# HKU-BAL/Clair3-RNA

Hardware: AMD Instinct MI355X
Metric: candidate sites/sec (tensor build + inference) (higher is better)
Workload: dtype f16 hi/lo split x3, f32 accumulate (fp32-equivalent); 1 GPU; synthetic ONT dRNA004 chr20 ~20x (BASELINE.json configs[1]); contig_len=64444167, chunks=13, channels=18, precision=f16x3, reads_per_rank=53937, exonic_bp_per_rank=1936903, parallelism=chunks sharded by contig, 1 rank(s), no collective, streams=2

## Files before the change

### clair3_rna_amd/csrc/net_kernels.hpp

```cpp
#pragma once
#include <hip/hip_runtime.h>
#include <mutex>
#include <chrono>
#include <type_traits>
#include <stdint.h>

#include <cmath>
#include <cstring>
#include <functional>
#include <string>
#include <vector>

#include "../../include/c3r.h"

namespace c3r {

typedef float floatx16 __attribute__((ext_vector_type(16)));
typedef float floatx4 __attribute__((ext_vector_type(4)));

constexpr int NET_H1 = 128;
constexpr int NET_H2 = 160;
constexpr int NET_T = C3R_WINDOW;
constexpr int NET_SITES = 32;
constexpr int LSTM_SB = 2;
constexpr int LSTM_SITES = NET_SITES * LSTM_SB;
#ifndef C3R_W8_PD
#define C3R_W8_PD 1
#endif
#ifndef C3R_W8_MAP
#define C3R_W8_MAP 0
#endif
#ifndef C3R_W8_PRIO
#define C3R_W8_PRIO 0
#endif
#ifndef C3R_DIR_ILV
#define C3R_DIR_ILV 1
#endif
#ifndef C3R_Y1_NT_LOAD
#define C3R_Y1_NT_LOAD 1
#endif
#ifndef C3R_Y1_NT_STORE
#define C3R_Y1_NT_STORE 1
#endif
#ifndef C3R_L2_SKIP0
#define C3R_L2_SKIP0 1
#endif
#define C3R_Y1_AUX (C3R_Y1_NT_LOAD ? 2 : 0)
template <class V, class P>
__device__ __forceinline__ void y1_store(V v, P p) {
    if constexpr (C3R_Y1_NT_STORE) __builtin_nontemporal_store(v, p);
    else *p = v;
}
constexpr int NET_FLAT = NET_T * 2 * NET_H2;
constexpr int NET_L4 = 128;

__device__ __forceinline__ float fast_sigmoid(float x) {
    return __builtin_amdgcn_rcpf(1.0f + __builtin_amdgcn_exp2f(-1.4426950408889634f * x));
}
__device__ __forceinline__ float fast_tanh(float x) {
    return fmaf(2.0f, __builtin_amdgcn_rcpf(1.0f + __builtin_amdgcn_exp2f(-2.8853900817779268f * x)), -1.0f);
}
__device__ __forceinline__ float gate_frac(float a, float b) {
    const float t = 1.0f + a;
    const float r = __builtin_amdgcn_rcpf(fmaf(t, b, t));
    return fmaf(-b, r, r);
}
__device__ __forceinline__ float cell_fence(float x) {
    asm("" : "+v"(x));
    return x;
}
typedef _Float16 half2v __attribute__((ext_vector_type(2)));
typedef float float2v __attribute__((ext_vector_type(2)));
__device__ __forceinline__ void split_h2(float h0, float h1, half2v &hi, half2v &lo, float &d0, float &d1) {
    asm("" : "+v"(h0));
    asm("" : "+v"(h1));
    const float2v h = {h0, h1};
    hi = __builtin_convertvector(h, half2v);
    asm("v_fma_mix_f32 %0, -%1, 1.0, %2 op_sel_hi:[1,1,0]" : "=v"(d0) : "v"(hi), "v"(h0));
    asm("v_fma_mix_f32 %0, -%1, 1.0, %2 op_sel:[1,0,0] op_sel_hi:[1,1,0]" : "=v"(d1) : "v"(hi), "v"(h1));
    const float2v d = {d0, d1};
    lo = __builtin_convertvector(d, half2v);
}
__device__ __forceinline__ float selu(float x) {
    const float scale = 1.0507009873554805f, alpha = 1.6732632423543772f;
    return x > 0.f ? scale * x : scale * alpha * (__expf(x) - 1.0f);
}

template <int INP, int CIN, int H, bool INT_IN, int SB = 2, int ABL = 0>
__global__ __launch_bounds__(256, (SB == 1 ? 2 : 1)) void k_lstm(const void *__restrict__ xin, const float4 *__restrict__ Wp,
                                                                  const float *__restrict__ bp, float *__restrict__ y, int n,
                                                                  const int32_t *__restrict__ row_idx = nullptr ,
                                                                  int x16 = 0 ) {
    constexpr int NGX = INP / 8;
    constexpr int NGH = H / 8;
    constexpr int NG = NGX + NGH;
    constexpr int HP = H + 4;
    constexpr int NBLK = 4 * H / 32;
    constexpr int NT = NBLK / 4;
    constexpr int WG_SITES = 32 * SB;
    static_assert(INP % 16 == 0 && H % 32 == 0, "shape: even k-group counts for the ping-pong pipeline");
    __shared__ __attribute__((aligned(16))) float hbuf[2][WG_SITES][HP];

    const int tid = threadIdx.x, lane = tid & 63, wave = tid >> 6;
    const int j = lane & 31, hh = lane >> 5;
    const int dir = blockIdx.y;
    const int site0 = blockIdx.x * WG_SITES;

    const float4 *wl = Wp + ((size_t)(dir * 4 + wave) * NG) * NT * 64 + lane;
    float bias_a[NT];
#pragma unroll
    for (int tt = 0; tt < NT; ++tt) bias_a[tt] = hh == 0 ? bp[((size_t)dir * NBLK + wave * NT + tt) * 32 + j] : 0.f;

    float cst[NT][SB][4];
#pragma unroll
    for (int tt = 0; tt < NT; ++tt)
#pragma unroll
        for (int sb = 0; sb < SB; ++sb)
#pragma unroll
            for (int q = 0; q < 4; ++q) cst[tt][sb][q] = 0.f;

    for (int i = tid; i < WG_SITES * HP; i += 256) (&hbuf[0][0][0])[i] = 0.f;
    __syncthreads();

    size_t xoff[SB];
#pragma unroll
    for (int sb = 0; sb < SB; ++sb) {
        int sj = site0 + 32 * sb + j;
        if (sj >= n) sj = n - 1;
        if (INT_IN && row_idx) sj = row_idx[sj];
        xoff[sb] = (size_t)sj * NET_T * CIN;
    }

    for (int step = 0; step < NET_T; ++step) {
        const int t = dir ? NET_T - 1 - step : step;
        const int cur = step & 1, nxt = cur ^ 1;

        auto ldx = [&](int g, float4 (&b)[SB]) {
#pragma unroll
            for (int sb = 0; sb < SB; ++sb) {
                if (ABL & 16) { b[sb] = make_float4(1.f, 0.5f, 0.25f, (float)g); continue; }
                if (INT_IN) {
                    const int k0 = 8 * g + 4 * hh;
                    if (x16) {
                        const int16_t *xp = (const int16_t *)xin + xoff[sb] + (size_t)t * CIN;
                        b[sb].x = (k0 + 0 < CIN) ? (float)xp[k0 + 0] : 0.f;
                        b[sb].y = (k0 + 1 < CIN) ? (float)xp[k0 + 1] : 0.f;
                        b[sb].z = (k0 + 2 < CIN) ? (float)xp[k0 + 2] : 0.f;
                        b[sb].w = (k0 + 3 < CIN) ? (float)xp[k0 + 3] : 0.f;
                    } else {
                        const int32_t *xp = (const int32_t *)xin + xoff[sb] + (size_t)t * CIN;
                        b[sb].x = (k0 + 0 < CIN) ? (float)xp[k0 + 0] : 0.f;
                        b[sb].y = (k0 + 1 < CIN) ? (float)xp[k0 + 1] : 0.f;
                        b[sb].z = (k0 + 2 < CIN) ? (float)xp[k0 + 2] : 0.f;
                        b[sb].w = (k0 + 3 < CIN) ? (float)xp[k0 + 3] : 0.f;
                    }
                } else {
                    b[sb] = *(const float4 *)((const float *)xin + xoff[sb] + (size_t)t * CIN + 8 * g + 4 * hh);
                }
            }
        };
        auto ldh = [&](int g, float4 (&b)[SB]) {
#pragma unroll
            for (int sb = 0; sb < SB; ++sb) b[sb] = *(const float4 *)&hbuf[cur][32 * sb + j][8 * g + 4 * hh];
        };
        auto ldw = [&](int g, float4 (&a)[NT]) {
            const float4 *wg = wl + (size_t)((ABL & 1) ? 0 : g) * NT * 64;
#pragma unroll
            for (int tt = 0; tt < NT; ++tt) a[tt] = wg[tt * 64];
        };

        floatx16 acc[NT][SB];
        {
            floatx16 z;
#pragma unroll
            for (int r = 0; r < 16; ++r) z[r] = 0.f;
#pragma unroll
            for (int tt = 0; tt < NT; ++tt)
#pragma unroll
                for (int sb = 0; sb < SB; ++sb) acc[tt][sb] = __builtin_amdgcn_mfma_f32_32x32x2f32(bias_a[tt], 1.0f, z, 0, 0, 0);
        }
#define C3R_MMA_K(comp)                                                                                              \
    _Pragma("unroll") for (int tt = 0; tt < NT; ++tt) _Pragma("unroll") for (int sb = 0; sb < SB; ++sb)             \
        acc[tt][sb] = __builtin_amdgcn_mfma_f32_32x32x2f32(a[tt].comp, b[sb].comp, acc[tt][sb], 0, 0, 0);
        auto mma = [&](const float4 (&a)[NT], const float4 (&b)[SB]) {
            C3R_MMA_K(x) C3R_MMA_K(y) C3R_MMA_K(z) C3R_MMA_K(w)
        };
#undef C3R_MMA_K
        float4 a0[NT], a1[NT], b0[SB], b1[SB];
#define C3R_FENCE() __builtin_amdgcn_sched_barrier(0)
        ldw(0, a0);
        ldx(0, b0);
#pragma unroll 1
        for (int g = 0; g + 2 < NGX; g += 2) {
            C3R_FENCE(); ldw(g + 1, a1); ldx(g + 1, b1); C3R_FENCE();
            mma(a0, b0);
            C3R_FENCE(); ldw(g + 2, a0); ldx(g + 2, b0); C3R_FENCE();
            mma(a1, b1);
        }
        C3R_FENCE(); ldw(NGX - 1, a1); ldx(NGX - 1, b1); C3R_FENCE();
        mma(a0, b0);
        C3R_FENCE(); ldw(NGX, a0); ldh(0, b0); C3R_FENCE();
        mma(a1, b1);
#pragma unroll 1
        for (int g = 0; g + 2 < NGH; g += 2) {
            C3R_FENCE(); ldw(NGX + g + 1, a1); ldh(g + 1, b1); C3R_FENCE();
            mma(a0, b0);
            C3R_FENCE(); ldw(NGX + g + 2, a0); ldh(g + 2, b0); C3R_FENCE();
            mma(a1, b1);
        }
        C3R_FENCE(); ldw(NG - 1, a1); ldh(NGH - 1, b1); C3R_FENCE();
        mma(a0, b0);
        mma(a1, b1);
        C3R_FENCE();
#undef C3R_FENCE
#pragma unroll
        for (int tt = 0; tt < NT; ++tt) {
#pragma unroll
            for (int sb = 0; sb < SB; ++sb) {
                float hq[4];
#pragma unroll
                for (int q = 0; q < 4; ++q) {
                    if (ABL & 2) { hq[q] = acc[tt][sb][4 * q] + acc[tt][sb][4 * q + 1] + acc[tt][sb][4 * q + 2] + acc[tt][sb][4 * q + 3]; continue; }
                    const float ig = fast_sigmoid(acc[tt][sb][4 * q + 0]);
                    const float fg = fast_sigmoid(acc[tt][sb][4 * q + 1]);
                    const float gg = fast_tanh(acc[tt][sb][4 * q + 2]);
                    const float og = fast_sigmoid(acc[tt][sb][4 * q + 3]);
                    const float c = fg * cst[tt][sb][q] + ig * gg;
                    cst[tt][sb][q] = c;
                    hq[q] = og * fast_tanh(c);
                }
                *(float4 *)&hbuf[nxt][32 * sb + j][8 * (wave * NT + tt) + 4 * hh] = make_float4(hq[0], hq[1], hq[2], hq[3]);
            }
        }
        if (!(ABL & 8)) __syncthreads();
        constexpr int HV = H / 4;
        if (!(ABL & 4))
        for (int f = tid; f < WG_SITES * HV; f += 256) {
            const int row = f / HV, c4 = f % HV;
            const int s = site0 + row;
            if (s < n) {
                const float4 v = *(const float4 *)&hbuf[nxt][row][4 * c4];
                *(float4 *)(y + ((size_t)s * NET_T + t) * (2 * H) + dir * H + 4 * c4) = v;
            }
        }
    }
}

typedef _Float16 half8 __attribute__((ext_vector_type(8)));
constexpr float WSCALE_LOG2 = 12.0f;
constexpr float WSCALE = 4096.0f;
constexpr float WUNSCALE = 1.0f / 4096.0f;

__device__ __forceinline__ float sigmoid_scaled(float acc) {
    return __builtin_amdgcn_rcpf(1.0f + __builtin_amdgcn_exp2f((-1.4426950408889634f * WUNSCALE) * acc));
}
__device__ __forceinline__ float tanh_scaled(float acc) {
    return fmaf(2.0f, __builtin_amdgcn_rcpf(1.0f + __builtin_amdgcn_exp2f((-2.8853900817779268f * WUNSCALE) * acc)), -1.0f);
}

template <int I, int N, class F>
__device__ __forceinline__ void static_for(F &&f) {
    if constexpr (I < N) { f(std::integral_constant<int, I>{}); static_for<I + 1, N>(f); }
}

template <int NM, int NV, int ND>
__device__ __forceinline__ void sched_interleave() {
    constexpr int K = (NM / (NV + ND + 1)) > 0 ? (NM / (NV + ND + 1)) : 1;
    if constexpr (NV > 0 && NM >= K) {
        __builtin_amdgcn_sched_group_barrier(0x008, K, 0);
        __builtin_amdgcn_sched_group_barrier(0x020, 1, 0);
        sched_interleave<NM - K, NV - 1, ND>();
    } else if constexpr (ND > 0 && NM >= K) {
        __builtin_amdgcn_sched_group_barrier(0x008, K, 0);
        __builtin_amdgcn_sched_group_barrier(0x100, 1, 0);
        sched_interleave<NM - K, NV, ND - 1>();
    } else if constexpr (NM > 0) {
        __builtin_amdgcn_sched_group_barrier(0x008, NM, 0);
    }
}


#ifndef C3R_W8_ASYNC
#define C3R_W8_ASYNC 1
#endif
__device__ __forceinline__ void lds_arrive(int *c) {
    __builtin_amdgcn_fence(__ATOMIC_RELEASE, "workgroup");
    if ((threadIdx.x & 63) == 0) atomicAdd(c, 1);
}
__device__ __forceinline__ void lds_wait(int *c, int target, int *tmo) {
    for (int it = 0; __atomic_load_n(c, __ATOMIC_RELAXED) < target; ++it) {
        if (it >= (1 << 24)) { if ((threadIdx.x & 63) == 0 && tmo) atomicOr(tmo, 1); break; }
        __builtin_amdgcn_s_sleep(1);
    }
    __builtin_amdgcn_fence(__ATOMIC_ACQUIRE, "workgroup");
}

#ifndef C3R_PROBE_Y1
#define C3R_PROBE_Y1 0
#endif
__host__ __device__ constexpr int w16_bias_row(int st, int q, int m) { return 8 * ((2 * q + st) & 3) + 4 * ((2 * q + st) >> 2) + m; }
template <int ABL = 0, bool RTS = false>
__global__ __launch_bounds__(512, 2) void k_lstm2_w16(const _Float16 *__restrict__ xin, const half8 *__restrict__ Wp,
                                                       const float *__restrict__ bp, int n, const half8 *__restrict__ W4p,
                                                       float *__restrict__ a4part, int nstride, float wsc_arg = WSCALE, float wun_arg = WUNSCALE, float wun4_arg = WUNSCALE,
                                                       int *tmo = nullptr ) {
    const float wsc = RTS ? wsc_arg : WSCALE, wun = RTS ? wun_arg : WUNSCALE, wun4 = RTS ? wun4_arg : WUNSCALE;
    constexpr int INP = 2 * NET_H1, H = NET_H2, NGX = INP / 32, NGH = H / 32, NG = NGX + NGH, NU = 2 * NG, HP = H + 8, NBLK = 4 * H / 32, NTQ = NBLK / 4;
    constexpr int SB = 4, WG_SITES = 16 * SB, KC = INP / 8, PD = C3R_W8_PD;
    static_assert(NTQ == 5 && NU == 26 && PD == 1, "3 + 2 tile split of a quarter, 26 (k-group, subtile) units, one unit of prefetch");
    __shared__ __attribute__((aligned(16))) _Float16 hb_hi[2][WG_SITES][HP];
    __shared__ __attribute__((aligned(16))) _Float16 hb_lo[2][WG_SITES][HP];
    __shared__ __attribute__((aligned(16))) _Float16 xs[2][KC][WG_SITES][8];
    __shared__ __attribute__((aligned(16))) float s_bias[NBLK][2][16];
    __shared__ int s_ctr[4];

    const int tid = threadIdx.x, lane = tid & 63;
    const int wave = __builtin_amdgcn_readfirstlane(tid >> 6);
    const int c16 = lane & 15, q4 = lane >> 4;
    const int sq = C3R_W8_MAP ? (wave >> 1) : (wave & 3);
    const bool heavy3 = C3R_W8_MAP ? !(wave & 1) : (wave < 4);
    const int dir = C3R_DIR_ILV ? blockIdx.x : blockIdx.y;
    const int site0 = (C3R_DIR_ILV ? blockIdx.y : blockIdx.x) * WG_SITES;
    const int ns = nstride ? nstride : n;
    const size_t plane_in = (size_t)ns * NET_T * INP;

    for (int i = tid; i < WG_SITES * HP; i += 512) { (&hb_hi[0][0][0])[i] = (_Float16)0.f; (&hb_lo[0][0][0])[i] = (_Float16)0.f; }
    for (int i = tid; i < NBLK * 32; i += 512) {
        const int T = i >> 5, st = (i >> 4) & 1, q = (i >> 2) & 3, m = i & 3;
        s_bias[T][st][4 * q + m] = wsc * bp[((size_t)dir * NBLK + T) * 32 + w16_bias_row(st, q, m)];
    }
    if (tid < 4) s_ctr[tid] = 0;

    int xsite = site0 + lane;
    if (xsite >= n) xsite = n - 1;
    auto dma_x = [&](int tt_) {
        typedef const _Float16 __attribute__((address_space(1))) *gp_t;
        typedef _Float16 __attribute__((address_space(3))) *lp_t;
#pragma unroll
        for (int r = 0; r < 2 * KC / 8; ++r) {
            const int row = wave * (2 * KC / 8) + r, pl = row / KC, kc = row % KC;
            const _Float16 *src = xin + (size_t)pl * plane_in + (((size_t)tt_ * KC + kc) * ns + xsite) * 8;
            __builtin_amdgcn_global_load_lds((gp_t)src, (lp_t)&xs[pl][kc][0][0], 16, 0, C3R_Y1_AUX);
        }
    };
    auto dma_x16 = [&](int tt_) {
        typedef const _Float16 __attribute__((address_space(1))) *gp_t;
        typedef _Float16 __attribute__((address_space(3))) *lp_t;
#pragma unroll
        for (int r = 0; r < 2 * KC / 4; ++r) {
            const int row = (wave & 3) * (2 * KC / 4) + r, pl = row / KC, kc = row % KC;
            const _Float16 *src = xin + (size_t)pl * plane_in + (((size_t)tt_ * KC + kc) * ns + xsite) * 8;
            __builtin_amdgcn_global_load_lds((gp_t)src, (lp_t)&xs[pl][kc][0][0], 16, 0, C3R_Y1_AUX);
        }
    };
    dma_x(dir ? NET_T - 1 : 0);
    asm volatile("s_waitcnt vmcnt(0)" ::: "memory");
    __syncthreads();

    auto body = [&](auto ntc, auto toffc, auto l4c) {
        constexpr int NT = decltype(ntc)::value, TOFF = decltype(toffc)::value;
        constexpr bool L4T = decltype(l4c)::value;
        constexpr int NTH = NT + (L4T ? 1 : 0);
        const half8 *wl = Wp + ((size_t)(dir * 4 + sq) * NU) * NTQ * 2 * 64 + (size_t)TOFF * 2 * 64;
        float cst[NT][2 * SB];
#pragma unroll
        for (int tt = 0; tt < NT; ++tt)
#pragma unroll
            for (int u = 0; u < 2 * SB; ++u) cst[tt][u] = 0.f;
        floatx4 facc[L4T ? 2 : 1][L4T ? SB : 1];
#pragma unroll
        for (int st = 0; st < (L4T ? 2 : 1); ++st)
#pragma unroll
            for (int sb = 0; sb < (L4T ? SB : 1); ++sb) {
#pragma unroll
                for (int r = 0; r < 4; ++r) {
                    float z = 0.f;
                    if constexpr (C3R_L2_SKIP0 && L4T) asm volatile("" : "+v"(z));
                    facc[st][sb][r] = z;
                }
            }

        typedef const half8 __attribute__((address_space(1))) *gptr_t;
        const uint32_t wlane = (uint32_t)lane;
        for (int step = 0; step < NET_T; ++step) {
            const int t = dir ? NET_T - 1 - step : step;
            const int tprev = step ? (dir ? t + 1 : t - 1) : t;
            const int cur = step & 1, nxt = cur ^ 1;

            auto ldx = [&](int g, half8 (&bh)[SB], half8 (&bl)[SB]) {
#pragma unroll
                for (int sb = 0; sb < SB; ++sb) {
                    if ((ABL & 32) && g > 0) continue;
                    bh[sb] = *(const half8 *)&xs[0][4 * g + q4][16 * sb + c16][0];
                    bl[sb] = *(const half8 *)&xs[1][4 * g + q4][16 * sb + c16][0];
                }
            };
            auto ldh = [&](int g, half8 (&bh)[SB], half8 (&bl)[SB]) {
#pragma unroll
                for (int sb = 0; sb < SB; ++sb) {
                    if (ABL & 32) continue;
                    bh[sb] = *(const half8 *)&hb_hi[cur][16 * sb + c16][32 * g + 8 * q4];
                    bl[sb] = *(const half8 *)&hb_lo[cur][16 * sb + c16][32 * g + 8 * q4];
                }
            };
            auto ldw = [&](int u, half8 (&ah)[NTH], half8 (&al)[NTH]) {
                gptr_t wg = (gptr_t)wl + (size_t)((ABL & 1) ? 0 : u) * NTQ * 2 * 64;
                asm volatile("" : "+s"(wg));
#pragma unroll
                for (int tt = 0; tt < NT; ++tt) {
                    if ((ABL & 16) && u > 0) continue;
                    ah[tt] = wg[(tt * 2 + 0) * 64 + wlane]; al[tt] = wg[(tt * 2 + 1) * 64 + wlane];
                }
                if constexpr (L4T) {
                    if (u >= 2 * NGX && !((ABL & 16) && u > 2 * NGX)) {
                        gptr_t w4 = (gptr_t)(W4p + (((size_t)(dir * NET_T + tprev) * 4 + sq) * 2 * NGH) * 2 * 64) + (size_t)(u - 2 * NGX) * 2 * 64;
                        asm volatile("" : "+s"(w4));
                        ah[NT] = w4[wlane]; al[NT] = w4[64 + wlane];
                    }
                }
            };

            if (C3R_W8_ASYNC && step > 0) lds_wait(&s_ctr[1], 4 * step, tmo);
            floatx4 acc[NT][2][SB];
#pragma unroll
            for (int tt = 0; tt < NT; ++tt)
#pragma unroll
                for (int st = 0; st < 2; ++st) {
                    const floatx4 b4 = *(const floatx4 *)&s_bias[sq * NTQ + TOFF + tt][st][4 * q4];
#pragma unroll
                    for (int sb = 0; sb < SB; ++sb) acc[tt][st][sb] = b4;
                }
            auto mma = [&](const half8 (&ah)[NTH], const half8 (&al)[NTH], const half8 (&bh)[SB], const half8 (&bl)[SB], auto stc, bool hpart) {
                constexpr int st = decltype(stc)::value;
#pragma unroll
                for (int tt = 0; tt < NT; ++tt)
#pragma unroll
                    for (int sb = 0; sb < SB; ++sb) acc[tt][st][sb] = __builtin_amdgcn_mfma_f32_16x16x32_f16(ah[tt], bh[sb], acc[tt][st][sb], 0, 0, 0);
                if (L4T && hpart) {
#pragma unroll
                    for (int sb = 0; sb < SB; ++sb) facc[L4T ? st : 0][L4T ? sb : 0] = __builtin_amdgcn_mfma_f32_16x16x32_f16(ah[L4T ? NT : 0], bh[sb], facc[L4T ? st : 0][L4T ? sb : 0], 0, 0, 0);
                }
#pragma unroll
                for (int tt = 0; tt < NT; ++tt)
#pragma unroll
                    for (int sb = 0; sb < SB; ++sb) acc[tt][st][sb] = __builtin_amdgcn_mfma_f32_16x16x32_f16(ah[tt], bl[sb], acc[tt][st][sb], 0, 0, 0);
                if (L4T && hpart) {
#pragma unroll
                    for (int sb = 0; sb < SB; ++sb) facc[L4T ? st : 0][L4T ? sb : 0] = __builtin_amdgcn_mfma_f32_16x16x32_f16(ah[L4T ? NT : 0], bl[sb], facc[L4T ? st : 0][L4T ? sb : 0], 0, 0, 0);
                }
#pragma unroll
                for (int tt = 0; tt < NT; ++tt)
#pragma unroll
                    for (int sb = 0; sb < SB; ++sb) acc[tt][st][sb] = __builtin_amdgcn_mfma_f32_16x16x32_f16(al[tt], bh[sb], acc[tt][st][sb], 0, 0, 0);
                if (L4T && hpart) {
#pragma unroll
                    for (int sb = 0; sb < SB; ++sb) facc[L4T ? st : 0][L4T ? sb : 0] = __builtin_amdgcn_mfma_f32_16x16x32_f16(al[L4T ? NT : 0], bh[sb], facc[L4T ? st : 0][L4T ? sb : 0], 0, 0, 0);
                }
            };
            half8 ah[2][NTH], al[2][NTH], bh[2][SB], bl[2][SB];
#define C3R_FENCE() __builtin_amdgcn_sched_barrier(0)
#define C3R_LOAD(U) do { ldw((U), ah[(U) % 2], al[(U) % 2]);                                                       \
                         if constexpr (((U) & 1) == 0) {                                                          \
                             if constexpr ((U) / 2 < NGX) ldx((U) / 2, bh[((U) / 2) % 2], bl[((U) / 2) % 2]);      \
                             else ldh((U) / 2 - NGX, bh[((U) / 2) % 2], bl[((U) / 2) % 2]); } } while (0)
#define C3R_STEP(U)                                                                                              \
    if constexpr ((U) < NU) {                                                                                     \
        C3R_FENCE();                                                                                              \
        if constexpr (C3R_W8_ASYNC && (U) + 1 == 2 * NGX) { lds_wait(&s_ctr[2], 8 * step, tmo); C3R_FENCE(); }    \
        if constexpr ((U) + 1 < NU) { C3R_LOAD((U) + 1); }                                                        \
        mma(ah[(U) % 2], al[(U) % 2], bh[((U) / 2) % 2], bl[((U) / 2) % 2], std::integral_constant<int, (U) & 1>{}, (U) >= 2 * NGX); \
        if constexpr ((U) + 1 < NU) {                                                                             \
            constexpr int NMM = ((U) >= 2 * NGX ? NTH : NT) * SB * 3;                                             \
            sched_interleave<NMM, ((U) + 1 >= 2 * NGX ? NTH : NT) * 2, (((U) & 1) ? SB * 2 : 0)>();                \
        }                                                                                                         \
        if constexpr ((U) == 2 * NGX - 1) {                                                                       \
            C3R_FENCE();                                                                                          \
            if constexpr (C3R_W8_ASYNC) lds_arrive(&s_ctr[0]); else __syncthreads();                              \
        }                                                                                                         \
    }
            static_assert(2 * NGX == 16, "the unit lists below: the x part ends with unit 15");
            C3R_LOAD(0);
            C3R_STEP(0) C3R_STEP(1) C3R_STEP(2) C3R_STEP(3) C3R_STEP(4) C3R_STEP(5) C3R_STEP(6) C3R_STEP(7) C3R_STEP(8) C3R_STEP(9)
            C3R_STEP(10) C3R_STEP(11) C3R_STEP(12) C3R_STEP(13) C3R_STEP(14) C3R_STEP(15)
            if (!C3R_L2_SKIP0 || step) {
            C3R_STEP(16) C3R_STEP(17) C3R_STEP(18)
            C3R_STEP(19) C3R_STEP(20) C3R_STEP(21) C3R_STEP(22) C3R_STEP(23) C3R_STEP(24) C3R_STEP(25)
            }
            C3R_FENCE();
#undef C3R_STEP
#undef C3R_LOAD
#undef C3R_FENCE
            if constexpr (C3R_W8_ASYNC) {
                if (!L4T && step + 1 < NET_T) { lds_wait(&s_ctr[0], 8 * (step + 1), tmo); dma_x16(dir ? NET_T - 2 - step : step + 1); }
            } else if (step + 1 < NET_T && !(ABL & 64)) dma_x(dir ? NET_T - 2 - step : step + 1);
#pragma unroll
            for (int tt = 0; tt < NT; ++tt) {
                __builtin_amdgcn_sched_barrier(0);
                constexpr int NC = 2 * SB;
                const float K1 = -1.4426950408889634f * wun, K2 = -2.8853900817779268f * wun;
                float cq[NC], ei[NC], ef[NC], eg[NC], eo[NC], hval[NC];
#pragma unroll
                for (int u = 0; u < NC; ++u) cq[u] = cst[tt][u];
                if (ABL & 2) {
#pragma unroll
                    for (int u = 0; u < NC; ++u) hval[u] = acc[tt][u / SB][u % SB][0] + acc[tt][u / SB][u % SB][1] + acc[tt][u / SB][u % SB][2] + acc[tt][u / SB][u % SB][3];
                } else {
#pragma unroll
                    for (int u = 0; u < NC; ++u) ei[u] = fminf(__builtin_amdgcn_exp2f(K1 * acc[tt][u / SB][u % SB][0]), 1e18f);
#pragma unroll
                    for (int u = 0; u < NC; ++u) ef[u] = __builtin_amdgcn_exp2f(K1 * acc[tt][u / SB][u % SB][1]);
#pragma unroll
                    for (int u = 0; u < NC; ++u) eg[u] = fminf(__builtin_amdgcn_exp2f(K2 * acc[tt][u / SB][u % SB][2]), 1e18f);
#pragma unroll
                    for (int u = 0; u < NC; ++u) eo[u] = __builtin_amdgcn_exp2f(K1 * acc[tt][u / SB][u % SB][3]);
#pragma unroll
                    for (int u = 0; u < NC; ++u) ei[u] = cell_fence(gate_frac(ei[u], eg[u]));
#pragma unroll
                    for (int u = 0; u < NC; ++u) ef[u] = __builtin_amdgcn_rcpf(1.0f + ef[u]);
#pragma unroll
                    for (int u = 0; u < NC; ++u) cq[u] = cell_fence(fmaf(ef[u], cq[u], ei[u]));
#pragma unroll
                    for (int u = 0; u < NC; ++u) eg[u] = fminf(__builtin_amdgcn_exp2f(-2.8853900817779268f * cq[u]), 1e18f);
#pragma unroll
                    for (int u = 0; u < NC; ++u) hval[u] = gate_frac(eo[u], eg[u]);
                }
#pragma unroll
                for (int u = 0; u < NC; ++u) cst[tt][u] = cq[u];
#pragma unroll
                for (int sb = 0; sb < SB; ++sb) {
                    half2v vh, vl;
                    float d0, d1;
                    split_h2(hval[sb], hval[SB + sb], vh, vl, d0, d1);
                    *(half2v *)&hb_hi[nxt][16 * sb + c16][8 * (sq * NTQ + TOFF + tt) + 2 * q4] = vh;
                    *(half2v *)&hb_lo[nxt][16 * sb + c16][8 * (sq * NTQ + TOFF + tt) + 2 * q4] = vl;
                }
            }
            if constexpr (C3R_W8_ASYNC) {
                lds_arrive(&s_ctr[2]);
                if (!L4T && step + 1 < NET_T) { asm volatile("s_waitcnt vmcnt(0)" ::: "memory"); lds_arrive(&s_ctr[1]); }
            } else {
            asm volatile("s_waitcnt vmcnt(0)" ::: "memory");
            __syncthreads();
            }
        }
        if constexpr (L4T) {
            if constexpr (C3R_W8_ASYNC) lds_wait(&s_ctr[2], 8 * NET_T, tmo);
            const int tl = dir ? 0 : NET_T - 1, hbuf = NET_T & 1;
            const half8 *w4 = W4p + (((size_t)(dir * NET_T + tl) * 4 + sq) * 2 * NGH) * 2 * 64 + lane;
#pragma unroll 1
            for (int g = 0; g < NGH; ++g) {
                half8 b_h[SB], b_l[SB];
#pragma unroll
                for (int sb = 0; sb < SB; ++sb) {
                    b_h[sb] = *(const half8 *)&hb_hi[hbuf][16 * sb + c16][32 * g + 8 * q4];
                    b_l[sb] = *(const half8 *)&hb_lo[hbuf][16 * sb + c16][32 * g + 8 * q4];
                }
#pragma unroll
                for (int st = 0; st < 2; ++st) {
                    const half8 a_h = w4[(size_t)((2 * g + st) * 2 + 0) * 64], a_l = w4[(size_t)((2 * g + st) * 2 + 1) * 64];
#pragma unroll
                    for (int sb = 0; sb < SB; ++sb) facc[st][sb] = __builtin_amdgcn_mfma_f32_16x16x32_f16(a_h, b_h[sb], facc[st][sb], 0, 0, 0);
#pragma unroll
                    for (int sb = 0; sb < SB; ++sb) facc[st][sb] = __builtin_amdgcn_mfma_f32_16x16x32_f16(a_h, b_l[sb], facc[st][sb], 0, 0, 0);
#pragma unroll
                    for (int sb = 0; sb < SB; ++sb) facc[st][sb] = __builtin_amdgcn_mfma_f32_16x16x32_f16(a_l, b_h[sb], facc[st][sb], 0, 0, 0);
                }
            }
#pragma unroll
            for (int sb = 0; sb < SB; ++sb) {
                const int sidx = site0 + 16 * sb + c16;
                if (sidx < n) {
#pragma unroll
                    for (int st = 0; st < 2; ++st) {
                        const floatx4 v = {facc[st][sb][0] * wun4, facc[st][sb][1] * wun4, facc[st][sb][2] * wun4, facc[st][sb][3] * wun4};
                        y1_store(v, (floatx4 *)(a4part + ((size_t)sidx * 2 + dir) * NET_L4 + 32 * sq + 16 * st + 4 * q4));
                    }
                }
            }
        }
    };
    if (C3R_W8_PRIO == 1 && heavy3) __builtin_amdgcn_s_setprio(1);
    if (C3R_W8_PRIO == 2 && !heavy3) __builtin_amdgcn_s_setprio(1);
    if (heavy3) body(std::integral_constant<int, 3>{}, std::integral_constant<int, 0>{}, std::false_type{});
    else body(std::integral_constant<int, 2>{}, std::integral_constant<int, 3>{}, std::true_type{});
}

__global__ __launch_bounds__(512, 2) void k_lstm2_mx(const _Float16 *__restrict__ xin, const half8 *__restrict__ Wp, const uint32_t *__restrict__ Wq,
                                                      const uint32_t *__restrict__ Wsc, const float *__restrict__ bp, int n,
                                                      const half8 *__restrict__ W4p, const uint32_t *__restrict__ W4q,
                                                      const uint32_t *__restrict__ W4sc, float *__restrict__ a4part, int nstride, int *tmo = nullptr) {
    constexpr int INP = 2 * NET_H1, H = NET_H2, NGX = INP / 16, NGH = H / 16, NG = NGX + NGH, HP = H + 8, NBLK = 4 * H / 32, NTQ = NBLK / 4;
    #ifndef C3R_MX_PD
#define C3R_MX_PD 1
#endif
#ifndef C3R_MX_EVEN_BURST
#define C3R_MX_EVEN_BURST 0
#endif
    constexpr int SB = 2, WG_SITES = 32 * SB, KC = INP / 8, PD = C3R_MX_PD;
    constexpr int NKB = NG / 2, NKBX = NGX / 2, NKBH = NGH / 2, NK4 = (NKB + 3) / 4, NK4L = (NKBH + 3) / 4;
    static_assert(NTQ == 5 && NG == 26 && NGX % 2 == 0 && NGH % 2 == 0, "3 + 2 tile split of a quarter, whole 32-k blocks");
    typedef int intx8 __attribute__((ext_vector_type(8)));
    typedef int intx4 __attribute__((ext_vector_type(4)));
    __shared__ __attribute__((aligned(16))) _Float16 hb_hi[2][WG_SITES][HP];
    __shared__ __attribute__((aligned(16))) intx4 hq[2][NKBH][2][2][WG_SITES];
    __shared__ __attribute__((aligned(16))) _Float16 xs[2][KC][WG_SITES][8];
    __shared__ int s_ctr[4];

    const int tid = threadIdx.x, lane = tid & 63, wave = tid >> 6;
    const int j = lane & 31, hh = lane >> 5;
    const int sq = wave & 3;
    const bool heavy3 = wave < 4;
    const int dir = C3R_DIR_ILV ? blockIdx.x : blockIdx.y;
    const int site0 = (C3R_DIR_ILV ? blockIdx.y : blockIdx.x) * WG_SITES;
    const int ns = nstride ? nstride : n;
    const size_t plane_in = (size_t)ns * NET_T * INP;

    for (int i = tid; i < WG_SITES * HP; i += 512) (&hb_hi[0][0][0])[i] = (_Float16)0.f;
    for (int i = tid; i < NKBH * 2 * 2 * WG_SITES; i += 512) (&hq[0][0][0][0][0])[i] = intx4{0, 0, 0, 0};
    if (tid < 4) s_ctr[tid] = 0;

    int xsite = site0 + lane;
    if (xsite >= n) xsite = n - 1;
    auto dma_x = [&](int tt_) {
        typedef const _Float16 __attribute__((address_space(1))) *gp_t;
        typedef _Float16 __attribute__((address_space(3))) *lp_t;
#pragma unroll
        for (int r = 0; r < 2 * KC / 8; ++r) {
            const int row = wave * (2 * KC / 8) + r, pl = row / KC, kc = row % KC;
            const _Float16 *src = xin + (size_t)pl * plane_in + (((size_t)tt_ * KC + kc) * ns + xsite) * 8;
            __builtin_amdgcn_global_load_lds((gp_t)src, (lp_t)&xs[pl][kc][0][0], 16, 0, C3R_Y1_AUX);
        }
    };
    auto dma_x16 = [&](int tt_) {
        typedef const _Float16 __attribute__((address_space(1))) *gp_t;
        typedef _Float16 __attribute__((address_space(3))) *lp_t;
#pragma unroll
        for (int r = 0; r < 2 * KC / 4; ++r) {
            const int row = (wave & 3) * (2 * KC / 4) + r, pl = row / KC, kc = row % KC;
            const _Float16 *src = xin + (size_t)pl * plane_in + (((size_t)tt_ * KC + kc) * ns + xsite) * 8;
            __builtin_amdgcn_global_load_lds((gp_t)src, (lp_t)&xs[pl][kc][0][0], 16, 0, C3R_Y1_AUX);
        }
    };
    dma_x(dir ? NET_T - 1 : 0);
    asm volatile("s_waitcnt vmcnt(0)" ::: "memory");
    __syncthreads();

    auto body = [&](auto ntc, auto toffc, auto l4c) {
        constexpr int NT = decltype(ntc)::value, TOFF = decltype(toffc)::value;
        constexpr bool L4T = decltype(l4c)::value;
        constexpr int NTH = NT + (L4T ? 1 : 0);
        const half8 *wl = Wp + ((size_t)(dir * 4 + sq) * NG) * NTQ * 2 * 64 + (size_t)TOFF * 2 * 64 + lane;
        const intx8 *wq = reinterpret_cast<const intx8 *>(Wq) + ((size_t)(dir * 4 + sq) * NKB * NTQ + TOFF) * 64 + lane;
        const uint32_t *wsc = Wsc + ((size_t)(dir * 4 + sq) * NK4 * NTQ + TOFF) * 64 + lane;
        typedef _Float16 half2v __attribute__((ext_vector_type(2)));
        unsigned bias_hl[NT];
#pragma unroll
        for (int tt = 0; tt < NT; ++tt) {
            const float bv = WSCALE * bp[((size_t)dir * NBLK + sq * NTQ + TOFF + tt) * 32 + j];
            half2v hl;
            hl[0] = (_Float16)bv;
            hl[1] = (_Float16)(bv - (float)hl[0]);
            bias_hl[tt] = hh == 0 ? __builtin_bit_cast(unsigned, hl) : 0u;
        }
        const half2v one2 = {(_Float16)1.f, (_Float16)1.f};
        const unsigned ones_b = hh == 0 ? __builtin_bit_cast(unsigned, one2) : 0u;
        const int sbc = hh ? 121 : 109;
        float cst[NT][SB][4];
#pragma unroll
        for (int tt = 0; tt < NT; ++tt)
#pragma unroll
            for (int sb = 0; sb < SB; ++sb)
#pragma unroll
                for (int q = 0; q < 4; ++q) cst[tt][sb][q] = 0.f;
        floatx16 facc[L4T ? SB : 1];
#pragma unroll
        for (int sb = 0; sb < (L4T ? SB : 1); ++sb)
#pragma unroll
            for (int r = 0; r < 16; ++r) facc[sb][r] = 0.f;

        typedef const half8 __attribute__((address_space(1))) *gptr_t;
        typedef const intx8 __attribute__((address_space(1))) *g8_t;
        typedef const uint32_t __attribute__((address_space(1))) *gs_t;
        auto ld_q = [&](g8_t p) {
            typedef const intx4 __attribute__((address_space(1))) *g4_t;
            const g4_t h = (g4_t)(p - lane) + lane;
            const intx4 lo = h[0], hi4 = h[64];
            return intx8{lo[0], lo[1], lo[2], lo[3], hi4[0], hi4[1], hi4[2], hi4[3]};
        };
        for (int step = 0; step < NET_T; ++step) {
            const int t = dir ? NET_T - 1 - step : step;
            const int tprev = step ? (dir ? t + 1 : t - 1) : t;
            const int cur = step & 1, nxt = cur ^ 1;

            if (C3R_W8_ASYNC && step > 0) lds_wait(&s_ctr[1], 4 * step, tmo);
            half8 ah[PD + 1][NTH], bh[PD + 1][SB];
            intx8 a8[NTH], b8[SB];
            int sc[NTH];
            auto load = [&](auto gc, half8 (&ahr)[NTH], half8 (&bhr)[SB]) {
                constexpr int G = decltype(gc)::value;
                uintptr_t wbase = (uintptr_t)wl;
                asm volatile("" : "+v"(wbase));
                const gptr_t wg = (gptr_t)wbase + (size_t)G * NTQ * 2 * 64;
#pragma unroll
                for (int tt = 0; tt < NT; ++tt) ahr[tt] = wg[(tt * 2 + 0) * 64];
                if constexpr (L4T && G >= NGX) {
                    uintptr_t w4base = (uintptr_t)(W4p + (((size_t)(dir * NET_T + tprev) * 4 + sq) * NGH) * 2 * 64 + lane);
                    asm volatile("" : "+v"(w4base));
                    ahr[NT] = ((gptr_t)w4base)[(size_t)(G - NGX) * 2 * 64];
                }
#pragma unroll
                for (int sb = 0; sb < SB; ++sb) {
                    if constexpr (G < NGX) bhr[sb] = *(const half8 *)&xs[0][2 * G + hh][32 * sb + j][0];
                    else bhr[sb] = *(const half8 *)&hb_hi[cur][32 * sb + j][16 * (G - NGX) + 8 * hh];
                }
                if constexpr ((G & 1) != 0) {
                    constexpr int KB = G / 2;
                    uintptr_t qbase = (uintptr_t)wq;
                    asm volatile("" : "+v"(qbase));
                    const g8_t qg = (g8_t)qbase + (size_t)KB * NTQ * 64;
#pragma unroll
                    for (int tt = 0; tt < NT; ++tt) a8[tt] = ld_q(qg + (size_t)tt * 64);
                    if constexpr (KB % 4 == 0) {
                        uintptr_t sbase = (uintptr_t)wsc;
                        asm volatile("" : "+v"(sbase));
                        const gs_t sg = (gs_t)sbase + (size_t)(KB / 4) * NTQ * 64;
#pragma unroll
                        for (int tt = 0; tt < NT; ++tt) sc[tt] = (int)sg[tt * 64];
                    }
                    if constexpr (L4T && KB >= NKBX) {
                        constexpr int KL = KB - NKBX;
                        uintptr_t q4 = (uintptr_t)(reinterpret_cast<const intx8 *>(W4q) + ((size_t)(dir * NET_T + tprev) * 4 + sq) * NKBH * 64 + lane);
                        asm volatile("" : "+v"(q4));
                        a8[L4T ? NT : 0] = ld_q((g8_t)q4 + (size_t)KL * 64);
                        if constexpr (KL % 4 == 0) {
                            uintptr_t s4 = (uintptr_t)(W4sc + ((size_t)(dir * NET_T + tprev) * 4 + sq) * NK4L * 64 + lane);
                            asm volatile("" : "+v"(s4));
                            sc[L4T ? NT : 0] = (int)((gs_t)s4)[(size_t)(KL / 4) * 64];
                        }
                    }
#pragma unroll
                    for (int sb = 0; sb < SB; ++sb) {
                        intx4 p0, p1;
                        if constexpr (KB < NKBX) {
                            p0 = *(const intx4 *)&xs[1][KB * 4 + 0 + hh][32 * sb + j][0];
                            p1 = *(const intx4 *)&xs[1][KB * 4 + 2 + hh][32 * sb + j][0];
                        } else {
                            p0 = hq[cur][KB - NKBX][0][hh][32 * sb + j];
                            p1 = hq[cur][KB - NKBX][1][hh][32 * sb + j];
                        }
                        b8[sb] = intx8{p0[0], p0[1], p0[2], p0[3], p1[0], p1[1], p1[2], p1[3]};
                    }
                }
            };

            floatx16 acc[NT][SB];
            {
                floatx16 z;
#pragma unroll
                for (int r = 0; r < 16; ++r) z[r] = 0.f;
                typedef unsigned uint4v __attribute__((ext_vector_type(4)));
                const uint4v bb = {ones_b, 0u, 0u, 0u};
#pragma unroll
                for (int tt = 0; tt < NT; ++tt) {
                    const uint4v ba = {bias_hl[tt], 0u, 0u, 0u};
#pragma unroll
                    for (int sb = 0; sb < SB; ++sb)
                        acc[tt][sb] = __builtin_amdgcn_mfma_f32_32x32x16_f16(__builtin_bit_cast(half8, ba), __builtin_bit_cast(half8, bb), z, 0, 0, 0);
                }
            }
            auto mma = [&](auto gc, const half8 (&ahr)[NTH], const half8 (&bhr)[SB]) {
                constexpr int G = decltype(gc)::value;
#pragma unroll
                for (int tt = 0; tt < NT; ++tt)
#pragma unroll
                    for (int sb = 0; sb < SB; ++sb) acc[tt][sb] = __builtin_amdgcn_mfma_f32_32x32x16_f16(ahr[tt], bhr[sb], acc[tt][sb], 0, 0, 0);
                if constexpr (L4T && G >= NGX) {
#pragma unroll
                    for (int sb = 0; sb < SB; ++sb) facc[L4T ? sb : 0] = __builtin_amdgcn_mfma_f32_32x32x16_f16(ahr[L4T ? NT : 0], bhr[sb], facc[L4T ? sb : 0], 0, 0, 0);
                }
                if constexpr ((G & 1) != 0) {
                    constexpr int KB = G / 2;
#pragma unroll
                    for (int tt = 0; tt < NT; ++tt)
#pragma unroll
                        for (int sb = 0; sb < SB; ++sb)
                            acc[tt][sb] = __builtin_amdgcn_mfma_scale_f32_32x32x64_f8f6f4(a8[tt], b8[sb], acc[tt][sb], 0, 0, KB % 4, sc[tt], 0, sbc);
                    if constexpr (L4T && KB >= NKBX) {
#pragma unroll
                        for (int sb = 0; sb < SB; ++sb)
                            facc[L4T ? sb : 0] = __builtin_amdgcn_mfma_scale_f32_32x32x64_f8f6f4(a8[L4T ? NT : 0], b8[sb], facc[L4T ? sb : 0], 0, 0, (KB - NKBX) % 4,
                                                                                                 sc[L4T ? NT : 0], 0, sbc);
                    }
                }
            };
#define C3R_FENCE() __builtin_amdgcn_sched_barrier(0)
#define C3R_STEP(G)                                                                                              \
    if constexpr ((G) < NG) {                                                                                     \
        C3R_FENCE();                                                                                              \
        if constexpr (C3R_W8_ASYNC && (G) + PD == NGX) { lds_wait(&s_ctr[2], 8 * step, tmo); C3R_FENCE(); }    \
        if constexpr (PD == 0 || (G) + PD < NG) { load(std::integral_constant<int, (G) + PD>{}, ah[((G) + PD) % (PD + 1)], bh[((G) + PD) % (PD + 1)]); } \
        mma(std::integral_constant<int, (G)>{}, ah[(G) % (PD + 1)], bh[(G) % (PD + 1)]);                          \
        if constexpr (PD > 0 && (G) + PD < NG && (((G) & 1) || !C3R_MX_EVEN_BURST)) {                              \
            constexpr int NMM = ((G) >= NGX ? NTH : NT) * SB * (((G) & 1) ? 2 : 1);                               \
            constexpr int NTL = ((G) + PD >= NGX ? NTH : NT);                                                     \
            sched_interleave<NMM, NTL * ((((G) + PD) & 1) ? 3 : 1), SB * ((((G) + PD) & 1) ? 3 : 1)>();           \
        }                                                                                                         \
        if constexpr ((G) == NGX - 1) {                                                                           \
            C3R_FENCE();                                                                                          \
            if constexpr (C3R_W8_ASYNC) lds_arrive(&s_ctr[0]); else __syncthreads();             \
        }                                                                                                         \
    }
            if constexpr (PD > 0) { load(std::integral_constant<int, 0>{}, ah[0], bh[0]); }
            C3R_STEP(0) C3R_STEP(1) C3R_STEP(2) C3R_STEP(3) C3R_STEP(4) C3R_STEP(5) C3R_STEP(6) C3R_STEP(7) C3R_STEP(8) C3R_STEP(9)
            C3R_STEP(10) C3R_STEP(11) C3R_STEP(12) C3R_STEP(13) C3R_STEP(14) C3R_STEP(15) C3R_STEP(16) C3R_STEP(17) C3R_STEP(18)
            C3R_STEP(19) C3R_STEP(20) C3R_STEP(21) C3R_STEP(22) C3R_STEP(23) C3R_STEP(24) C3R_STEP(25)
            C3R_FENCE();
#undef C3R_STEP
#undef C3R_FENCE
            if constexpr (C3R_W8_ASYNC) {
                if (!L4T && step + 1 < NET_T) { lds_wait(&s_ctr[0], 8 * (step + 1), tmo); dma_x16(dir ? NET_T - 2 - step : step + 1); }
            } else if (step + 1 < NET_T) dma_x(dir ? NET_T - 2 - step : step + 1);
#pragma unroll
            for (int tt = 0; tt < NT; ++tt) {
                __builtin_amdgcn_sched_barrier(0);
                constexpr int NU = 4 * SB;
                constexpr float K1 = -1.4426950408889634f * WUNSCALE, K2 = -2.8853900817779268f * WUNSCALE;
                float cq[NU], ei[NU], ef[NU], eg[NU], eo[NU], hval[NU];
#pragma unroll
                for (int u = 0; u < NU; ++u) cq[u] = cst[tt][u >> 2][u & 3];
#pragma unroll
                for (int u = 0; u < NU; ++u) ei[u] = fminf(__builtin_amdgcn_exp2f(K1 * acc[tt][u >> 2][4 * (u & 3) + 0]), 1e18f);
#pragma unroll
                for (int u = 0; u < NU; ++u) ef[u] = __builtin_amdgcn_exp2f(K1 * acc[tt][u >> 2][4 * (u & 3) + 1]);
#pragma unroll
                for (int u = 0; u < NU; ++u) eg[u] = fminf(__builtin_amdgcn_exp2f(K2 * acc[tt][u >> 2][4 * (u & 3) + 2]), 1e18f);
#pragma unroll
                for (int u = 0; u < NU; ++u) eo[u] = __builtin_amdgcn_exp2f(K1 * acc[tt][u >> 2][4 * (u & 3) + 3]);
#pragma unroll
                for (int u = 0; u < NU; ++u) ei[u] = cell_fence(gate_frac(ei[u], eg[u]));
#pragma unroll
                for (int u = 0; u < NU; ++u) ef[u] = __builtin_amdgcn_rcpf(1.0f + ef[u]);
#pragma unroll
                for (int u = 0; u < NU; ++u) cq[u] = cell_fence(fmaf(ef[u], cq[u], ei[u]));
#pragma unroll
                for (int u = 0; u < NU; ++u) eg[u] = fminf(__builtin_amdgcn_exp2f(-2.8853900817779268f * cq[u]), 1e18f);
#pragma unroll
                for (int u = 0; u < NU; ++u) hval[u] = gate_frac(eo[u], eg[u]);
                const int T = sq * NTQ + TOFF + tt;
#pragma unroll
                for (int sb = 0; sb < SB; ++sb) {
#pragma unroll
                    for (int q = 0; q < 4; ++q) cst[tt][sb][q] = cq[4 * sb + q];
                    typedef _Float16 half4 __attribute__((ext_vector_type(4)));
                    half2v vh01, vh23, vl01, vl23;
                    float lo[4];
                    split_h2(hval[4 * sb + 0], hval[4 * sb + 1], vh01, vl01, lo[0], lo[1]);
                    split_h2(hval[4 * sb + 2], hval[4 * sb + 3], vh23, vl23, lo[2], lo[3]);
                    const half4 vh = __builtin_shufflevector(vh01, vh23, 0, 1, 2, 3);
#pragma unroll
                    for (int q = 0; q < 4; ++q) lo[q] *= 262144.f;
                    *(half4 *)&hb_hi[nxt][32 * sb + j][8 * T + 4 * hh] = vh;
                    int w_lo = __builtin_amdgcn_cvt_pk_fp8_f32(lo[0], lo[1], 0, false);
                    w_lo = __builtin_amdgcn_cvt_pk_fp8_f32(lo[2], lo[3], w_lo, true);
                    int w_hi = __builtin_amdgcn_cvt_pk_fp8_f32(hval[4 * sb + 0] * 64.f, hval[4 * sb + 1] * 64.f, 0, false);
                    w_hi = __builtin_amdgcn_cvt_pk_fp8_f32(hval[4 * sb + 2] * 64.f, hval[4 * sb + 3] * 64.f, w_hi, true);
                    {
                    reinterpret_cast<int *>(&hq[nxt][T >> 2][0][(T & 3) >> 1][32 * sb + j])[2 * (T & 1) + hh] = w_lo;
                    reinterpret_cast<int *>(&hq[nxt][T >> 2][1][(T & 3) >> 1][32 * sb + j])[2 * (T & 1) + hh] = w_hi;
                    }
                }
// ... 962 lines not shown
```

Baseline: 9.073 million sites/s.

## Reschedule LSTM layer-2 weight loads and defer L4 projection to step end

Hoists the first unit's weight load for the next timestep to the end of the current step, so it overlaps the gate nonlinearity work. The L4 (flatten-dense) contribution is moved out of the recurrent MFMA stream into a separate block after each step's sync, with its own prefetch and h-buffer double buffering. The final tail L4 pass also gets a small ring of prefetched weights. This is meant to hide global-memory latency in the recurrent critical path. The cost is higher register pressure and an extra LDS counter wait when async mode is on.

```diff
diff --git a/clair3_rna_amd/csrc/net_kernels.hpp b/clair3_rna_amd/csrc/net_kernels.hpp
--- a/clair3_rna_amd/csrc/net_kernels.hpp
+++ b/clair3_rna_amd/csrc/net_kernels.hpp
@@ -45,6 +45,15 @@
 #ifndef C3R_L2_SKIP0
 #define C3R_L2_SKIP0 1
 #endif
+#ifndef C3R_L2_PRE0
+#define C3R_L2_PRE0 1
+#endif
+#ifndef C3R_L2_L4_LATE
+#define C3R_L2_L4_LATE 1
+#endif
+#ifndef C3R_L2_TAIL_RING
+#define C3R_L2_TAIL_RING 1
+#endif
 #define C3R_Y1_AUX (C3R_Y1_NT_LOAD ? 2 : 0)
 template <class V, class P>
 __device__ __forceinline__ void y1_store(V v, P p) {
@@ -360,7 +369,10 @@
     auto body = [&](auto ntc, auto toffc, auto l4c) {
         constexpr int NT = decltype(ntc)::value, TOFF = decltype(toffc)::value;
         constexpr bool L4T = decltype(l4c)::value;
-        constexpr int NTH = NT + (L4T ? 1 : 0);
+        constexpr bool L4R = L4T && !C3R_L2_L4_LATE;
+        constexpr bool L4L = L4T && C3R_L2_L4_LATE;
+        constexpr int NTH = NT + (L4R ? 1 : 0);
+        constexpr int L4PRE = 2;
         const half8 *wl = Wp + ((size_t)(dir * 4 + sq) * NU) * NTQ * 2 * 64 + (size_t)TOFF * 2 * 64;
         float cst[NT][2 * SB];
 #pragma unroll
@@ -382,6 +394,17 @@
 
         typedef const half8 __attribute__((address_space(1))) *gptr_t;
         const uint32_t wlane = (uint32_t)lane;
+        auto ldwx = [&](int u, half8 (&ah)[NTH], half8 (&al)[NTH]) {
+            gptr_t wg = (gptr_t)wl + (size_t)((ABL & 1) ? 0 : u) * NTQ * 2 * 64;
+            asm volatile("" : "+s"(wg));
+#pragma unroll
+            for (int tt = 0; tt < NT; ++tt) {
+                if ((ABL & 16) && u > 0) continue;
+                ah[tt] = wg[(tt * 2 + 0) * 64 + wlane]; al[tt] = wg[(tt * 2 + 1) * 64 + wlane];
+            }
+        };
+        half8 ah[2][NTH], al[2][NTH], bh[2][SB], bl[2][SB];
+        if constexpr (C3R_L2_PRE0) ldwx(0, ah[0], al[0]);
         for (int step = 0; step < NET_T; ++step) {
             const int t = dir ? NET_T - 1 - step : step;
             const int tprev = step ? (dir ? t + 1 : t - 1) : t;
@@ -404,20 +427,19 @@
                 }
             };
             auto ldw = [&](int u, half8 (&ah)[NTH], half8 (&al)[NTH]) {
-                gptr_t wg = (gptr_t)wl + (size_t)((ABL & 1) ? 0 : u) * NTQ * 2 * 64;
-                asm volatile("" : "+s"(wg));
-#pragma unroll
-                for (int tt = 0; tt < NT; ++tt) {
-                    if ((ABL & 16) && u > 0) continue;
-                    ah[tt] = wg[(tt * 2 + 0) * 64 + wlane]; al[tt] = wg[(tt * 2 + 1) * 64 + wlane];
-                }
-                if constexpr (L4T) {
+                ldwx(u, ah, al);
+                if constexpr (L4R) {
                     if (u >= 2 * NGX && !((ABL & 16) && u > 2 * NGX)) {
                         gptr_t w4 = (gptr_t)(W4p + (((size_t)(dir * NET_T + tprev) * 4 + sq) * 2 * NGH) * 2 * 64) + (size_t)(u - 2 * NGX) * 2 * 64;
                         asm volatile("" : "+s"(w4));
-                        ah[NT] = w4[wlane]; al[NT] = w4[64 + wlane];
+                        ah[L4R ? NT : 0] = w4[wlane]; al[L4R ? NT : 0] = w4[64 + wlane];
                     }
                 }
+            };
+            auto ldw4 = [&](int u, half8 &a_h, half8 &a_l) {
+                gptr_t w4 = (gptr_t)(W4p + (((size_t)(dir * NET_T + tprev) * 4 + sq) * 2 * NGH) * 2 * 64) + (size_t)u * 2 * 64;
+                asm volatile("" : "+s"(w4));
+                a_h = w4[wlane]; a_l = w4[64 + wlane];
             };
 
             if (C3R_W8_ASYNC && step > 0) lds_wait(&s_ctr[1], 4 * step, tmo);
@@ -436,28 +458,27 @@
                 for (int tt = 0; tt < NT; ++tt)
 #pragma unroll
                     for (int sb = 0; sb < SB; ++sb) acc[tt][st][sb] = __builtin_amdgcn_mfma_f32_16x16x32_f16(ah[tt], bh[sb], acc[tt][st][sb], 0, 0, 0);
-                if (L4T && hpart) {
-#pragma unroll
-                    for (int sb = 0; sb < SB; ++sb) facc[L4T ? st : 0][L4T ? sb : 0] = __builtin_amdgcn_mfma_f32_16x16x32_f16(ah[L4T ? NT : 0], bh[sb], facc[L4T ? st : 0][L4T ? sb : 0], 0, 0, 0);
+                if (L4R && hpart) {
+#pragma unroll
+                    for (int sb = 0; sb < SB; ++sb) facc[L4T ? st : 0][L4T ? sb : 0] = __builtin_amdgcn_mfma_f32_16x16x32_f16(ah[L4R ? NT : 0], bh[sb], facc[L4T ? st : 0][L4T ? sb : 0], 0, 0, 0);
                 }
 #pragma unroll
                 for (int tt = 0; tt < NT; ++tt)
 #pragma unroll
                     for (int sb = 0; sb < SB; ++sb) acc[tt][st][sb] = __builtin_amdgcn_mfma_f32_16x16x32_f16(ah[tt], bl[sb], acc[tt][st][sb], 0, 0, 0);
-                if (L4T && hpart) {
-#pragma unroll
-                    for (int sb = 0; sb < SB; ++sb) facc[L4T ? st : 0][L4T ? sb : 0] = __builtin_amdgcn_mfma_f32_16x16x32_f16(ah[L4T ? NT : 0], bl[sb], facc[L4T ? st : 0][L4T ? sb : 0], 0, 0, 0);
+                if (L4R && hpart) {
+#pragma unroll
+                    for (int sb = 0; sb < SB; ++sb) facc[L4T ? st : 0][L4T ? sb : 0] = __builtin_amdgcn_mfma_f32_16x16x32_f16(ah[L4R ? NT : 0], bl[sb], facc[L4T ? st : 0][L4T ? sb : 0], 0, 0, 0);
                 }
 #pragma unroll
                 for (int tt = 0; tt < NT; ++tt)
 #pragma unroll
                     for (int sb = 0; sb < SB; ++sb) acc[tt][st][sb] = __builtin_amdgcn_mfma_f32_16x16x32_f16(al[tt], bh[sb], acc[tt][st][sb], 0, 0, 0);
-                if (L4T && hpart) {
-#pragma unroll
-                    for (int sb = 0; sb < SB; ++sb) facc[L4T ? st : 0][L4T ? sb : 0] = __builtin_amdgcn_mfma_f32_16x16x32_f16(al[L4T ? NT : 0], bh[sb], facc[L4T ? st : 0][L4T ? sb : 0], 0, 0, 0);
+                if (L4R && hpart) {
+#pragma unroll
+                    for (int sb = 0; sb < SB; ++sb) facc[L4T ? st : 0][L4T ? sb : 0] = __builtin_amdgcn_mfma_f32_16x16x32_f16(al[L4R ? NT : 0], bh[sb], facc[L4T ? st : 0][L4T ? sb : 0], 0, 0, 0);
                 }
             };
-            half8 ah[2][NTH], al[2][NTH], bh[2][SB], bl[2][SB];
 #define C3R_FENCE() __builtin_amdgcn_sched_barrier(0)
 #define C3R_LOAD(U) do { ldw((U), ah[(U) % 2], al[(U) % 2]);                                                       \
                          if constexpr (((U) & 1) == 0) {                                                          \
@@ -479,7 +500,8 @@
         }                                                                                                         \
     }
             static_assert(2 * NGX == 16, "the unit lists below: the x part ends with unit 15");
-            C3R_LOAD(0);
+            if constexpr (C3R_L2_PRE0) ldx(0, bh[0], bl[0]);
+            else { C3R_LOAD(0); }
             C3R_STEP(0) C3R_STEP(1) C3R_STEP(2) C3R_STEP(3) C3R_STEP(4) C3R_STEP(5) C3R_STEP(6) C3R_STEP(7) C3R_STEP(8) C3R_STEP(9)
             C3R_STEP(10) C3R_STEP(11) C3R_STEP(12) C3R_STEP(13) C3R_STEP(14) C3R_STEP(15)
             if (!C3R_L2_SKIP0 || step) {
@@ -490,9 +512,16 @@
 #undef C3R_STEP
 #undef C3R_LOAD
 #undef C3R_FENCE
+            if constexpr (C3R_W8_ASYNC && C3R_L2_L4_LATE) lds_wait(&s_ctr[3], 4 * step, tmo);
             if constexpr (C3R_W8_ASYNC) {
                 if (!L4T && step + 1 < NET_T) { lds_wait(&s_ctr[0], 8 * (step + 1), tmo); dma_x16(dir ? NET_T - 2 - step : step + 1); }
             } else if (step + 1 < NET_T && !(ABL & 64)) dma_x(dir ? NET_T - 2 - step : step + 1);
+            if (C3R_L2_PRE0 && step + 1 < NET_T) ldwx(0, ah[0], al[0]);
+            half8 a4h[L4L ? 2 * NGH : 1], a4l[L4L ? 2 * NGH : 1];
+            if constexpr (L4L) {
+#pragma unroll
+                for (int u = 0; u < L4PRE; ++u) ldw4(u, a4h[u], a4l[u]);
+            }
 #pragma unroll
             for (int tt = 0; tt < NT; ++tt) {
                 __builtin_amdgcn_sched_barrier(0);
@@ -542,8 +571,65 @@
             asm volatile("s_waitcnt vmcnt(0)" ::: "memory");
             __syncthreads();
             }
-        }
-        if constexpr (L4T) {
+            if constexpr (L4L) {
+                if (step) {
+                    half8 b4h[2][SB], b4l[2][SB];
+                    __builtin_amdgcn_sched_barrier(0);
+#pragma unroll
+                    for (int u = L4PRE; u < 2 * NGH; ++u) ldw4(u, a4h[u], a4l[u]);
+                    ldh(0, b4h[0], b4l[0]);
+#pragma unroll
+                    for (int u = 0; u < 2 * NGH; ++u) {
+                        const int g = u / 2, st = u & 1;
+                        __builtin_amdgcn_sched_barrier(0);
+                        if (st == 0 && g + 1 < NGH) ldh(g + 1, b4h[(g + 1) % 2], b4l[(g + 1) % 2]);
+#pragma unroll
+                        for (int sb = 0; sb < SB; ++sb) facc[L4T ? st : 0][L4T ? sb : 0] = __builtin_amdgcn_mfma_f32_16x16x32_f16(a4h[L4L ? u : 0], b4h[g % 2][sb], facc[L4T ? st : 0][L4T ? sb : 0], 0, 0, 0);
+#pragma unroll
+                        for (int sb = 0; sb < SB; ++sb) facc[L4T ? st : 0][L4T ? sb : 0] = __builtin_amdgcn_mfma_f32_16x16x32_f16(a4h[L4L ? u : 0], b4l[g % 2][sb], facc[L4T ? st : 0][L4T ? sb : 0], 0, 0, 0);
+#pragma unroll
+                        for (int sb = 0; sb < SB; ++sb) facc[L4T ? st : 0][L4T ? sb : 0] = __builtin_amdgcn_mfma_f32_16x16x32_f16(a4l[L4L ? u : 0], b4h[g % 2][sb], facc[L4T ? st : 0][L4T ? sb : 0], 0, 0, 0);
+                    }
+                    __builtin_amdgcn_sched_barrier(0);
+                }
+                if constexpr (C3R_W8_ASYNC) lds_arrive(&s_ctr[3]);
+            }
+        }
+        if constexpr (L4T && C3R_L2_TAIL_RING) {
+            const int tl = dir ? 0 : NET_T - 1, hbuf = NET_T & 1;
+            gptr_t w4t = (gptr_t)(W4p + (((size_t)(dir * NET_T + tl) * 4 + sq) * 2 * NGH) * 2 * 64);
+            half8 a_h[2], a_l[2];
+            auto lda = [&](int u, half8 &h_, half8 &l_) {
+                gptr_t p = w4t + (size_t)u * 2 * 64;
+                asm volatile("" : "+s"(p));
+                h_ = p[wlane]; l_ = p[64 + wlane];
+            };
+            lda(0, a_h[0], a_l[0]);
+            lda(1, a_h[1], a_l[1]);
+            if constexpr (C3R_W8_ASYNC) lds_wait(&s_ctr[2], 8 * NET_T, tmo);
+#pragma unroll 1
+            for (int g = 0; g < NGH; ++g) {
+                half8 b_h[SB], b_l[SB];
+#pragma unroll
+                for (int sb = 0; sb < SB; ++sb) {
+                    b_h[sb] = *(const half8 *)&hb_hi[hbuf][16 * sb + c16][32 * g + 8 * q4];
+                    b_l[sb] = *(const half8 *)&hb_lo[hbuf][16 * sb + c16][32 * g + 8 * q4];
+                }
+                const int gn = g + 1 < NGH ? g + 1 : NGH - 1;
+#pragma unroll
+                for (int st = 0; st < 2; ++st) {
+                    __builtin_amdgcn_sched_barrier(0);
+#pragma unroll
+                    for (int sb = 0; sb < SB; ++sb) facc[st][sb] = __builtin_amdgcn_mfma_f32_16x16x32_f16(a_h[st], b_h[sb], facc[st][sb], 0, 0, 0);
+#pragma unroll
+                    for (int sb = 0; sb < SB; ++sb) facc[st][sb] = __builtin_amdgcn_mfma_f32_16x16x32_f16(a_h[st], b_l[sb], facc[st][sb], 0, 0, 0);
+#pragma unroll
+                    for (int sb = 0; sb < SB; ++sb) facc[st][sb] = __builtin_amdgcn_mfma_f32_16x16x32_f16(a_l[st], b_h[sb], facc[st][sb], 0, 0, 0);
+                    __builtin_amdgcn_sched_barrier(0);
+                    lda(2 * gn + st, a_h[st], a_l[st]);
+                }
+            }
+        } else if constexpr (L4T) {
             if constexpr (C3R_W8_ASYNC) lds_wait(&s_ctr[2], 8 * NET_T, tmo);
             const int tl = dir ? 0 : NET_T - 1, hbuf = NET_T & 1;
             const half8 *w4 = W4p + (((size_t)(dir * NET_T + tl) * 4 + sq) * 2 * NGH) * 2 * 64 + lane;
@@ -566,6 +652,8 @@
                     for (int sb = 0; sb < SB; ++sb) facc[st][sb] = __builtin_amdgcn_mfma_f32_16x16x32_f16(a_l, b_h[sb], facc[st][sb], 0, 0, 0);
                 }
             }
+        }
+        if constexpr (L4T) {
 #pragma unroll
             for (int sb = 0; sb < SB; ++sb) {
                 const int sidx = site0 + 16 * sb + c16;
```

Result: slower. 8.921 million sites/s (-1.7%).
